# 1dayac/spades_for_blackbird

Hardware: AMD Instinct MI355X
Metric: distinct k-mers/sec (k=21, 150 bp synthetic reads, count only) (higher is better)
Workload: dtype u64

## Files before the change

### spades_for_blackbird_amd/csrc/bbk_internal.h

```cpp
#pragma once

#include <hip/hip_runtime.h>

#include <cstdint>
#include <cstdio>
#include <cstdlib>
#include <map>
#include <memory>
#include <string>
#include <type_traits>
#include <utility>
#include <vector>

#include "../../include/bbk.h"

namespace bbk {

void set_error(const char *fmt, ...);
const char *get_error();

struct Error {
    int code;
};

// ... 97 lines not shown
    int num_cus = 256;
    int num_xcds = 8;
    struct Pending {
        hipEvent_t a, b;
        std::string family;
        double bytes;
    };
    std::vector<Pending> pending;
    std::map<std::string, bbk::FamilyStat> stats;
    void resolve_pending();
    void add_stat(const char *name, double value) {
        if (!profiling) return;
        bbk::FamilyStat &f = stats[name];
        f.launches += 1;
        f.bytes += value;
    }
    void *pinned[2] = {nullptr, nullptr};
    size_t pinned_bytes = 0;
    void *plan_pinned = nullptr;
    size_t plan_pinned_bytes = 0;
    size_t mem_free = 0;
    uint64_t mem_free_mapped_now = ~0ull, mem_free_mapped_total = ~0ull;
    double superk_dup = 0;
};

namespace bbk {

struct KernelTimer {
    bbk_ctx *ctx;
    hipEvent_t a = nullptr, b = nullptr;
    std::string family;
    double bytes;
    KernelTimer(bbk_ctx *c, const char *fam, double algorithmic_bytes = 0) : ctx(c), family(fam), bytes(algorithmic_bytes) {
        if (ctx->profiling) {
            BBK_HIP(hipEventCreate(&a));
            BBK_HIP(hipEventCreate(&b));
            BBK_HIP(hipEventRecord(a, ctx->stream));
        }
    }
    ~KernelTimer() {
        if (a) {
            (void)hipEventRecord(b, ctx->stream);
            ctx->pending.push_back({a, b, family, bytes});
        }
    }
};
// ... 11 lines not shown
                  Args... args) {
    if (lds)
        BBK_HIP(hipFuncSetAttribute(reinterpret_cast<const void *>(fn), hipFuncAttributeMaxDynamicSharedMemorySize,
                                    (int)lds));
    KernelTimer t(ctx, name, bytes);
    hipLaunchKernelGGL(fn, dim3(grid), dim3(threads), lds, ctx->stream, args...);
    check_launch(name);
}

template <class F>
void dispatch_w(unsigned W, F &&f) {
    switch (W) {
        case 1: f(std::integral_constant<int, 1>{}); break;
        case 2: f(std::integral_constant<int, 2>{}); break;
        case 3: f(std::integral_constant<int, 3>{}); break;
        case 4: f(std::integral_constant<int, 4>{}); break;
        default: BBK_REQUIRE(false, BBK_ERR_ARG, "unsupported key width %u", W);
    }
}

inline void stream_wait(bbk_ctx *ctx) {
    ctx->add_stat("stat_host_waits", 1);
    BBK_HIP(hipStreamSynchronize(ctx->stream));
}

inline void d2h_sync(bbk_ctx *ctx, void *dst, const void *src, size_t bytes) {
    BBK_HIP(hipMemcpyAsync(dst, src, bytes, hipMemcpyDeviceToHost, ctx->stream));
    BBK_HIP(hipStreamSynchronize(ctx->stream));
}

inline uint64_t env_u64(const char *v, uint64_t unset) { return v ? strtoull(v, nullptr, 10) : unset; }

inline unsigned words_of(unsigned k) { return (k + 31) >> 5; }

#define BBK_GID() ((((uint64_t)blockIdx.y * gridDim.x) + blockIdx.x) * blockDim.x + threadIdx.x)
inline dim3 grid_blocks(uint64_t blocks) {
    constexpr uint64_t kMaxX = 1ull << 21;
    if (blocks <= kMaxX) return dim3((unsigned)(blocks ? blocks : 1));
    return dim3((unsigned)kMaxX, (unsigned)((blocks + kMaxX - 1) / kMaxX));
}

template <class K, class... Args>
void launch_items(bbk_ctx *ctx, const char *name, K fn, uint64_t n_threads, Args... args) {
    hipLaunchKernelGGL(fn, grid_blocks((n_threads + 255) / 256), dim3(256), 0, ctx->stream, args...);
    check_launch(name);
}
// ... 36 lines not shown
    const uint64_t *d_words = nullptr;
    const uint64_t *d_woff = nullptr;
    const uint32_t *d_len = nullptr;
    bbk::DevBuf own_words, own_woff, own_len;
};

struct bbk_kmerset {
    unsigned k = 0, W = 0;
    unsigned flags = 0;
    uint64_t n = 0;
    uint64_t instances = 0;
    bbk::DevBuf keys;
    bbk::DevBuf counts;
    bool has_counts = false;
    bool sorted = true;
    bool ref_order = false;
};

namespace bbk {

uint64_t exclusive_scan_u64(bbk_ctx *ctx, const uint64_t *in, uint64_t *out, uint64_t n);
void exclusive_scan2_u64(bbk_ctx *ctx, const uint64_t *in0, uint64_t *out0, const uint64_t *in1, uint64_t *out1,
                         uint64_t n, uint64_t totals[2]);
enum { SCAN_U64 = 0, SCAN_U32_FLAGGED = 1, SCAN_SLOT_FILL = 2, SCAN_READ_UNITS = 3 };
struct ScanSrc {
    const void *p;
    uint32_t kind, stride, cap;
    const uint64_t *woff = nullptr;
    uint32_t *unordered = nullptr;
};
void exclusive_scan_enqueue(bbk_ctx *ctx, int narr, const ScanSrc *src, uint64_t *const *out, uint64_t n,
                            uint64_t *d_total, bool tail, std::vector<DevBuf> &keep);

struct ReadPlan {
    DevBuf coff;
    uint64_t kmers = 0, units = 0;
    void run(bbk_ctx *ctx, const bbk_reads *rd, unsigned k, unsigned C, uint32_t *d_unordered);
};

struct PassDesc {
    int kind;
    int word;
    int shift;
    int bits;
    unsigned nb;
};

std::vector<PassDesc> key_passes(unsigned k);

void sort_records(bbk_ctx *ctx, int W, void *keys, void *keys_tmp, uint32_t *vals, uint32_t *vals_tmp, uint64_t n,
                  const std::vector<PassDesc> &passes);
void partition_records(bbk_ctx *ctx, int W, const void *src, void *dst, const uint32_t *vsrc, uint32_t *vdst, uint64_t n,
                       const PassDesc &pd, uint64_t *h_digit_totals = nullptr);
// ... 37 lines not shown
```

### spades_for_blackbird_amd/csrc/block_scan.h

```cpp
#pragma once

#include <hip/hip_runtime.h>

#include <cstdint>

namespace bbk {

constexpr int kThreads = 256;
constexpr int kWaves = kThreads / 64;

__device__ inline uint32_t wave_incl_scan(uint32_t v) {
    const int lane = threadIdx.x & 63;
#pragma unroll
    for (int d = 1; d < 64; d <<= 1) {
        uint32_t t = __shfl_up(v, d, 64);
        if (lane >= d) v += t;
    }
    return v;
}

__device__ inline uint32_t block_excl_scan(uint32_t v, uint32_t *smem_waves , uint32_t *total) {
    const int lane = threadIdx.x & 63, wave = threadIdx.x >> 6;
    uint32_t incl = wave_incl_scan(v);
    if (lane == 63) smem_waves[wave] = incl;
    __syncthreads();
    uint32_t base = 0, tot = 0;
#pragma unroll
    for (int w = 0; w < kWaves; ++w) {
        uint32_t s = smem_waves[w];
        if (w < wave) base += s;
        tot += s;
    }
    __syncthreads();
    *total = tot;
    return base + incl - v;
}

}
```

### spades_for_blackbird_amd/csrc/context.hip

```cpp
#include <hip/hip_runtime.h>

#include <fcntl.h>
#include <unistd.h>

#include <algorithm>
#include <cstdarg>
#include <cstring>

#include "bbk_internal.h"

namespace bbk {

static thread_local char g_err[1024] = "";
void set_error(const char *fmt, ...) {
    va_list ap;
    va_start(ap, fmt);
    vsnprintf(g_err, sizeof(g_err), fmt, ap);
    va_end(ap);
}
const char *get_error() { return g_err; }

hipError_t copy_async(void *dst, const void *src, size_t bytes, hipMemcpyKind kind, hipStream_t stream) {
    if (bytes == 0) return hipSuccess;
    return hipMemcpyAsync(dst, src, bytes, kind, stream);
// ... 150 lines not shown
                (void)hipMemsetAsync(d_mask, 0, 4, c->stream);
                hipLaunchKernelGGL(k_xcd_probe, dim3(4096), dim3(64), 0, c->stream, d_mask);
                if (hipMemcpyAsync(&h_mask, d_mask, 4, hipMemcpyDeviceToHost, c->stream) == hipSuccess &&
                    hipStreamSynchronize(c->stream) == hipSuccess && h_mask)
                    c->num_xcds = __builtin_popcount(h_mask);
                (void)hipFree(d_mask);
            }
            (void)hipGetLastError();
        }
        *out = c;
    });
}

int bbk_ctx_destroy(bbk_ctx *ctx) {
    if (!ctx) return BBK_OK;
    (void)hipSetDevice(ctx->device);
    ctx->resolve_pending();
    if (ctx->stream) (void)hipStreamSynchronize(ctx->stream);
    bbk::pool_trim(ctx->device);
    if (getenv("BBK_VERBOSE")) bbk::pool_report();
    if (ctx->pinned[0]) (void)hipHostFree(ctx->pinned[0]);
    if (ctx->pinned[1]) (void)hipHostFree(ctx->pinned[1]);
    if (ctx->plan_pinned) (void)hipHostFree(ctx->plan_pinned);
    if (ctx->own_stream && ctx->stream) (void)hipStreamDestroy(ctx->stream);
    delete ctx;
    return BBK_OK;
}

int bbk_ctx_set_stream(bbk_ctx *ctx, void *hip_stream) {
    return bbk::guarded([&] {
        BBK_REQUIRE(ctx != nullptr, BBK_ERR_ARG, "bbk_ctx_set_stream: ctx is NULL");
        BBK_HIP(hipSetDevice(ctx->device));
        BBK_HIP(hipStreamSynchronize(ctx->stream));
        if (ctx->own_stream && ctx->stream) BBK_HIP(hipStreamDestroy(ctx->stream));
        ctx->stream = reinterpret_cast<hipStream_t>(hip_stream);
        ctx->own_stream = false;
    });
}

int bbk_ctx_trim(bbk_ctx *ctx) {
    return bbk::guarded([&] {
        BBK_REQUIRE(ctx != nullptr, BBK_ERR_ARG, "bbk_ctx_trim: ctx is NULL");
        BBK_HIP(hipSetDevice(ctx->device));
        BBK_HIP(hipStreamSynchronize(ctx->stream));
        bbk::pool_trim(ctx->device);
    });
// ... 70 lines not shown
```

### spades_for_blackbird_amd/csrc/msd.hip

```cpp
#include <hip/hip_runtime.h>

#include <algorithm>
#include <chrono>
#include <cmath>
#include <cstdio>
#include <cstdlib>
#include <cstring>
#include <optional>
#include <type_traits>
#include <utility>
#include <vector>

#include "bbk_internal.h"
#include "kmer_ops.h"
#include "msd.h"
#include "msd.h"

#include "msd_part.h"
#include "msd_bucket.h"
#include "msd_narrow_a.h"
#include "msd_stage_b.h"

namespace bbk {

// ... 282 lines not shown
        uint64_t *ctl_total() const { return reinterpret_cast<uint64_t *>(ctl_at(kCtlTotal)); }
        uint64_t h_total() const {
            uint64_t t;
            memcpy(&t, h_ctl + kCtlTotal, 8);
            return t;
        }
        ReadSrc S{}, Sh{};
        TileMap M1{}, M2{};
        PartLevel L1{}, L2{};
        DevBuf spill_k, spill_v;
        DevBuf hist1, cur1, bufA, valA;
        uint32_t n32 = 0;
        std::vector<uint32_t> h1, off1, tstart, snb2, sbin, hsub, fill1;
        std::vector<uint32_t> over_seg;
        uint32_t nbuckets = 0, ntiles2 = 0, nwg2 = 0;
        bool narrow_b = false;
        uint32_t *stage = nullptr;
        DevBuf layout_d;
        uint32_t *seg_tile = nullptr, *seg_off = nullptr, *seg_nb2 = nullptr, *seg_bin = nullptr, *seg_size = nullptr,
                 *xstart_d = nullptr;
        DevBuf desc2, desc2h, hist2, boff, bufB, valB;
        std::vector<uint32_t> xstart;
        DevBuf dcount, slot_off, bseg, bbase, flag_ids;
        DevBuf bperm, pfill;
        DevBuf c64, d64;
        bool d64_scanned = false;
        std::vector<DevBuf> scan_keep;
        BucketArgs A{};
        bool direct = false;
        uint32_t ctr[4] = {0, 0, 0, 0};
        std::vector<uint32_t> flagged, hd, hb;
        std::vector<uint32_t> big;
        uint32_t hbo[2] = {0, 0};
        MsdOutput extra;
        uint64_t novf = 0;

        Pass(MsdRunner &r, const MsdInput &i, MsdOutput &o, const Sel &s, Dst d)
            : R(r), ctx(r.ctx), in(i), out(o), sel(s), dst(d), from_reads(i.rd != nullptr),
              has_val(i.with_mask || i.vals != nullptr), ranged(s.span != 0), has_dst(d.keys != nullptr),
              out_vals(r.op != MSD_OP_NONE), need_vbuf(has_val || out_vals), verbose(r.knobs.verbose) {}

        double rec_bytes(uint64_t n) const { return (double)n * (rec + (has_val ? 4 : 0)); }
        uint32_t *vals_or_null(DevBuf &b) const { return has_val ? b.as<uint32_t>() : nullptr; }

        Outcome run(uint64_t *n_records = nullptr) {
            ctl.alloc(kCtlWords * 4);
            BBK_HIP(hipMemsetAsync(ctl.p, 0, kCtlWords * 4, ctx->stream));
// ... 441 lines not shown
                if constexpr (W == 1)
                    R.template launch_part<false, false, false, true>("k_part_l2", (double)N * (rec + 4), nwg2,
                                                                        bufA.as<Key<W>>(), nullptr, M2, L2, nullptr,
                                                                        hist2.as<uint32_t>(), bufB.as<Key<W>>(), nullptr);
            } else {
                R.template scatter_keys<false>(has_val, "k_part_l2", 2.0 * rec_bytes(N), nwg2, bufA.as<Key<W>>(), valA.as<uint32_t>(), M2,
                               L2, hist2.as<uint32_t>(), bufB.as<Key<W>>(), valB.as<uint32_t>());
            }
        }

        std::optional<Outcome> first_pass() {
            dcount.alloc((size_t)nbuckets * 4 + 16);
            A = BucketArgs{boff.as<uint32_t>(), dcount.as<uint32_t>(), nullptr, (int)R.k,
                           verbose ? ctl_at(kCtlDbg) : nullptr, P.slots ? P.cap2 : 0u, P.slots ? P.stride2 : 0u,
                           hist2.as<uint32_t>(), nullptr, nullptr, nullptr, ~0ull, R.knobs.once.hash_max_probes, nullptr};
            direct = (!P.slots || P.kslots) && R.assume_distinct && (R.dmode == MSD_KEYS || R.dmode == MSD_REF) &&
                     !R.knobs.no_direct;
            if (P.kslots) {
                c64.alloc(((size_t)nbuckets + 1) * 8);
                uint64_t *const so = c64.as<uint64_t>();
                slot_off.alloc(((size_t)nbuckets + 1) * 4 + 16);
                if (P.late_tag) {
                    bbase.alloc(((size_t)nbuckets + 1) * 8);
                    bperm.alloc(((size_t)nbuckets + 1) * 4);
                    pfill.alloc(((size_t)nbuckets + 1) * 4);
                    R.launch_plan(k_bucket_base_lt, "k_bucket_base_lt", nbuckets, (const uint32_t *)seg_nb2,
                                  (const uint32_t *)seg_bin, P.nb1, nbuckets, 2 * (int)R.expand_k - 10, (int)R.expand_k,
                                  bbase.as<uint64_t>(), bperm.as<uint32_t>());
                    R.launch_plan(k_lt_fill_perm, "k_lt_fill_perm", nbuckets, hist2.as<uint32_t>(), bperm.as<uint32_t>(),
                                  nbuckets, P.stride2, P.cap2, pfill.as<uint32_t>());
                    const ScanSrc src{pfill.p, SCAN_U32_FLAGGED, 0u, 0u};
                    exclusive_scan_enqueue(ctx, 1, &src, &so, nbuckets, ctl_total(), false, scan_keep);
                    R.launch_plan(k_lt_unperm, "k_lt_unperm", nbuckets, c64.as<uint64_t>(), bperm.as<uint32_t>(), nbuckets,
                                  slot_off.as<uint32_t>());
                } else {
                    const ScanSrc src{hist2.p, SCAN_SLOT_FILL, P.stride2, P.cap2};
                    exclusive_scan_enqueue(ctx, 1, &src, &so, nbuckets, ctl_total(), false, scan_keep);
                    R.launch_plan(k_scan_to_u32, "k_scan_to_u32", (uint64_t)nbuckets + 1, c64.as<uint64_t>(),
                                  (uint64_t)nbuckets, 0ull, (const uint64_t *)ctl_total(), slot_off.as<uint32_t>());
                }
                A.out_off = slot_off.as<uint32_t>();
            }
            if (direct) {
                if (!has_dst) {
                    out.keys.alloc(N * rec + 16);
                    if (out_vals) out.vals.alloc(N * 4 + 16);
                }
                A.sorted_keys = has_dst ? dst.keys : out.keys.p;
                A.sorted_vals = has_dst ? dst.vals : out.vals.as<uint32_t>();
                A.dup_flag = ctl_at(kCtlDup);
                A.strip_mask = R.strip_mask;
            }
            launch_buckets();
            flag_ids.alloc((size_t)kFlagCap * 4);
            if (P.hslots && !direct) {
                d64.alloc(((size_t)nbuckets + 1) * 8);
                const ScanSrc src{dcount.p, SCAN_U32_FLAGGED, 0u, 0u};
                uint64_t *const so = d64.as<uint64_t>();
                exclusive_scan_enqueue(ctx, 1, &src, &so, nbuckets, ctl_total(), false, scan_keep);
                d64_scanned = true;
            }
            fetch_flags();
            if (P.kslots && h_total() != N) {
                if (verbose) fprintf(stderr, "[bbk] msd key slots: %llu of %llu records placed, exact mode\n",
                                     (unsigned long long)h_total(), (unsigned long long)N);
                out.keys.release();
                out.vals.release();
                return give_up_key_slots();
            }
            if (!direct) return std::nullopt;
            if (ctr[2] == 0 && ctr[3] == 0 && (!P.kslots || ctr[0] == 0)) {
                out.n = N;
                out.nbuckets = 0;
                out.overflow_buckets = 0;
                if (P.kslots && verbose)
                    fprintf(stderr, "[bbk] msd key slots N=%llu buckets=%u: ordered without histograms\n",
                            (unsigned long long)N, nbuckets);
                return Outcome::Done;
            }
            if (P.kslots) {
// ... 31 lines not shown
            } else if (narrow_b) {
                if constexpr (W == 1) {
                    BBK_REQUIRE(direct, BBK_ERR_INTERNAL, "4-byte stage-B records need the direct output");
                    if (!P.late_tag) bbase.alloc(((size_t)nbuckets + 1) * 8);
                    if (nbuckets) {
                        if (!P.late_tag)
                            R.launch_plan(k_bucket_base, "k_bucket_base", nbuckets, (const uint32_t *)seg_nb2,
                                          (const uint32_t *)seg_bin, P.nb1, nbuckets, P.b1, R.w0bits(), bbase.as<uint64_t>());
                        constexpr int NT = BktCfg<1>::NT, IT = BktCfg<1>::ITEMS;
                        const bool wide = A.slot_cap != 0 && A.slot_stride % 4 == 0;
                        R.launch(wide ? k_bucket_dist_nb<NT, IT, true> : k_bucket_dist_nb<NT, IT, false>, "k_bucket_dist",
                                 (double)N * (4 + rec), nbuckets, NT, bucket_dist_nb_smem<NT, IT>(), bufB.as<uint32_t>(),
                                 bbase.as<uint64_t>(), A);
                    }
                }
            } else {
                R.template bucket_dispatch<false>(nbuckets, bufB.as<Key<W>>(), valB.as<uint32_t>(), A, rec_bytes(N));
            }
        }

        void fetch_flags() {
            uint32_t *d_flag_n = P.slots ? ctl_at(kCtlSpill) + 2 : ctl_at(kCtlFlagN);
            if (!P.slots) BBK_HIP(hipMemsetAsync(d_flag_n, 0, 16, ctx->stream));
            R.launch_plan(k_flagged, "k_flagged", nbuckets, dcount.as<uint32_t>(), nbuckets, flag_ids.as<uint32_t>(), kFlagCap,
                          d_flag_n);
            BBK_HIP(hipMemcpyAsync(h_ctl, ctl.p, kCtlWords * 4, hipMemcpyDeviceToHost, ctx->stream));
            stream_wait(ctx);
            if (P.slots) memcpy(ctr, h_ctl + kCtlSpill, 12);
            else ctr[2] = h_ctl[kCtlFlagN];
            if (direct) ctr[3] = h_ctl[kCtlDup];
        }

        std::optional<Outcome> overflow() {
            const uint32_t n_flag = ctr[2];
            if (n_flag > kFlagCap) {
                if (verbose) fprintf(stderr, "[bbk] msd: %u buckets overflow\n", n_flag);
                return P.slots ? Outcome::SlotsGaveUp : Outcome::Declined;
            }
            flagged.resize(n_flag);
            if (n_flag) {
                BBK_HIP(hipMemcpyAsync(flagged.data(), flag_ids.p, (size_t)n_flag * 4, hipMemcpyDeviceToHost, ctx->stream));
                stream_wait(ctx);
                std::sort(flagged.begin(), flagged.end());
            }
            const bool exact_check = !P.slots && (n_flag || verbose);
            if (exact_check) {
                hd.resize(nbuckets);
                hb.resize((size_t)nbuckets + 1);
// ... 675 lines not shown
```

### spades_for_blackbird_amd/csrc/msd_part.h

```cpp
#pragma once

namespace bbk {

#ifndef BBK_KEYS_TILE
#define BBK_KEYS_TILE 8192
#endif
#ifndef BBK_KEYS_THREADS
#define BBK_KEYS_THREADS 512
#endif
template <int W>
struct PartCfg {
    static constexpr int TILE = (W == 1) ? BBK_KEYS_TILE : (W == 2 ? 4096 : 2048);
    static constexpr int THREADS = BBK_KEYS_THREADS;
    static constexpr int ITEMS = TILE / THREADS;
};
constexpr int kRdThreads = 1024;
constexpr int kRdHistThreads = 512;
constexpr int kRdSlots = 1024;
constexpr int kRdWords = 2048;
template <int W>
struct RdCfg {
    static constexpr int CH = (W == 1) ? 8 : (W == 2 ? 4 : 2);
    static constexpr int TILE = kRdThreads * CH;
};
// ... 154 lines not shown
        const uint64_t rem = M.n - T.begin;
        T.count = rem < (uint64_t)tile_size ? (uint32_t)rem : tile_size;
        T.nb = L.nb1;
        T.gbin0 = 0;
    }
    return T;
}

#ifdef BBK_PHASE_PROF
__device__ unsigned long long g_phase[6][8];
#define BBK_PH(kind, ph, t_prev)                                                   \
    do {                                                                           \
        if (threadIdx.x == 0) {                                                    \
            const unsigned long long t_now = clock64();                            \
            atomicAdd(&g_phase[kind][ph], t_now - t_prev);                         \
            t_prev = t_now;                                                        \
        }                                                                          \
    } while (0)
#else
#define BBK_PH(kind, ph, t_prev) \
    do {                         \
    } while (0)
#endif

__device__ __forceinline__ uint32_t wave_scan_incl(uint32_t v) {
    v += (uint32_t)__builtin_amdgcn_update_dpp(0, (int)v, 0x111, 0xf, 0xf, false);
    v += (uint32_t)__builtin_amdgcn_update_dpp(0, (int)v, 0x112, 0xf, 0xf, false);
    v += (uint32_t)__builtin_amdgcn_update_dpp(0, (int)v, 0x114, 0xf, 0xf, false);
    v += (uint32_t)__builtin_amdgcn_update_dpp(0, (int)v, 0x118, 0xf, 0xf, false);
    v += (uint32_t)__builtin_amdgcn_update_dpp(0, (int)v, 0x142, 0xa, 0xf, false);
    v += (uint32_t)__builtin_amdgcn_update_dpp(0, (int)v, 0x143, 0xc, 0xf, false);
    return v;
}

template <int NW>
__device__ __forceinline__ void wave_totals(const uint32_t *tmp, int lane, int wave, uint32_t &before, uint32_t &total) {
    static_assert(NW <= 16, "one DPP row");
    const uint32_t v = lane < NW ? tmp[lane] : 0u;
    uint32_t inc = v;
    if (NW > 1) inc += (uint32_t)__builtin_amdgcn_update_dpp(0, (int)inc, 0x111, 0xf, 0xf, false);
    if (NW > 2) inc += (uint32_t)__builtin_amdgcn_update_dpp(0, (int)inc, 0x112, 0xf, 0xf, false);
    if (NW > 4) inc += (uint32_t)__builtin_amdgcn_update_dpp(0, (int)inc, 0x114, 0xf, 0xf, false);
    if (NW > 8) inc += (uint32_t)__builtin_amdgcn_update_dpp(0, (int)inc, 0x118, 0xf, 0xf, false);
    total = (uint32_t)__builtin_amdgcn_readlane((int)inc, NW - 1);
    before = (uint32_t)__builtin_amdgcn_readlane((int)(inc - v), __builtin_amdgcn_readfirstlane(wave));
}

template <int W, int ITEMS, int THREADS, int MAXB, bool HAS_VAL, bool NOUT = false>
__device__ __forceinline__ void part_tail(const Key<W> (&keys)[ITEMS], const uint32_t (&vals)[ITEMS],
                                          const uint32_t (&binrank)[ITEMS], uint32_t *lhist, uint32_t *lstart,
                                          uint32_t *goff, uint32_t *scan_tmp, Key<W> *stage, uint32_t *vstage,
                                          uint32_t nb, uint64_t gbin0, const PartLevel &L,
                                          uint32_t *__restrict__ cursor, Key<W> *__restrict__ out,
                                          uint32_t *__restrict__ vout, int prof_kind = 0,
                                          unsigned long long t_prev = 0) {
    const int tid = threadIdx.x;
// ... 503 lines not shown
```

### spades_for_blackbird_amd/csrc/msd_stage_b.h

```cpp
#pragma once

#include "msd_bucket_tail.h"

namespace bbk {

__global__ void k_bucket_base(const uint32_t *__restrict__ seg_nb2, const uint32_t *__restrict__ seg_bin, uint32_t nseg,
                              uint32_t nbuckets, int b1, int w0bits, uint64_t *__restrict__ base) {
    const uint32_t g = blockIdx.x * blockDim.x + threadIdx.x;
    if (g >= nbuckets) return;
    const uint32_t lo = last_le(seg_bin, nseg, g);
    const uint64_t P = 1ull << (32 - b1), nb = seg_nb2[lo], j = g - seg_bin[lo];
    const uint64_t p = lo * P + (j * P + nb - 1) / nb;
    base[g] = w0bits > 32 ? p << (w0bits - 32) : 0ull;
}

template <int NT, int ITEMS, bool WIDE>
__global__ __launch_bounds__(NT) __attribute__((amdgpu_waves_per_eu(8, 8))) void k_bucket_dist_nb(const uint32_t *__restrict__ buf, const uint64_t *__restrict__ base,
                                                       BucketArgs A) {
    constexpr int CAP = NT * ITEMS;
    constexpr int NWAVES = NT / 64;
    constexpr int DB = DistBins<1, 0>::N;
    constexpr int BPT = DB / NT;
    extern __shared__ __attribute__((aligned(16))) unsigned char smem[];
    uint32_t *bins = reinterpret_cast<uint32_t *>(smem);
// ... 527 lines not shown
    }
#pragma unroll
    for (int i = 0; i < ITEMS; ++i) asm volatile("" : "+v"(lo[i]));
#pragma unroll
    for (int i = 0; i < ITEMS; ++i) {
        Key<1> x;
        x.w[0] = segbits | lo[i];
        const uint32_t tag = (uint32_t)__umul64hi(xxh3_64<1>(x), 16ull);
        const uint32_t b = tag * nsub + __umulhi(lo[i] << (32 - lobits), nsub);
        const bool valid = (uint32_t)i * NT + tid < count;
        if (valid) atomicAdd(&S.lhist[b], 1u);
        const uint32_t b16 = valid ? b : 0xFFFFu;
        if (i & 1) bins[i >> 1] |= b16 << 16;
        else bins[i >> 1] = b16;
    }
    __syncthreads();
    const uint64_t slot_end = (uint64_t)(gbin0 + tid) * L.slot_stride + L.slot_cap;
    mark_tail<NT * ITEMS, ITEMS, false>(
        S, lo, tid, nb, &cursor[gbin0 + tid], slot_end, (uint32_t)segbits, L, out, nullptr,
        [&](int i) { return lt_bin<ITEMS>(bins, i); }, [](int) { return 0u; },
        [&](uint32_t, uint32_t rec) { return lt_tagged(sgm, rec, lobits, k); }, []() {});
}

__global__ void k_bucket_base_lt(const uint32_t *__restrict__ seg_nb2, const uint32_t *__restrict__ seg_bin, uint32_t nseg,
                                 uint32_t nbuckets, int lobits, int k, uint64_t *__restrict__ base,
                                 uint32_t *__restrict__ perm) {
    const uint32_t g = blockIdx.x * blockDim.x + threadIdx.x;
    if (g >= nbuckets) return;
    const uint32_t lo = last_le(seg_bin, nseg, g);
    const uint32_t nsub = seg_nb2[lo] >> 4, r = g - seg_bin[lo], tag = r / nsub, j = r - tag * nsub;
    const uint64_t q = (((uint64_t)j << lobits) + nsub - 1u) / nsub;
    base[g] = ((uint64_t)tag << (2 * k)) | ((uint64_t)lo << lobits) | q;
    perm[g] = tag * (nbuckets >> 4) + (seg_bin[lo] >> 4) + j;
}

__global__ void k_lt_fill_perm(const uint32_t *__restrict__ cursor, const uint32_t *__restrict__ perm, uint32_t n,
                               uint32_t stride, uint32_t cap, uint32_t *__restrict__ fill) {
    const uint32_t g = blockIdx.x * blockDim.x + threadIdx.x;
    if (g >= n) return;
    const uint32_t c = cursor[g] - g * stride;
    fill[perm[g]] = c < cap ? c : cap;
}

__global__ void k_lt_unperm(const uint64_t *__restrict__ scanned, const uint32_t *__restrict__ perm, uint32_t n,
                            uint32_t *__restrict__ out_off) {
    const uint32_t g = blockIdx.x * blockDim.x + threadIdx.x;
    if (g < n) out_off[g] = (uint32_t)scanned[perm[g]];
}

__global__ void k_view_recanon_lt(const uint32_t *__restrict__ in, const uint32_t *__restrict__ seg_off,
                                  const uint32_t *__restrict__ seg_size, int sub_shift, int k, uint64_t *__restrict__ out,
                                  uint64_t cap, uint32_t *__restrict__ count) {
    const uint32_t o = seg_off[blockIdx.x], n = seg_size[blockIdx.x];
    const uint64_t segbits = (uint64_t)(blockIdx.x >> sub_shift) << (2 * k - 10);
    const int lane = threadIdx.x & 63;
    for (uint32_t i0 = 0; i0 < n; i0 += blockDim.x) {
        const uint32_t i = i0 + threadIdx.x;
        Key<1> x;
        x.w[0] = 0;
        bool keep = false;
        if (i < n) {
            x.w[0] = segbits | in[o + i];
            keep = !kmer_less_nucl<1>(kmer_rc<1>(x, k), x);
        }
        const uint64_t bal = __ballot(keep);
        uint32_t base = 0;
        if (lane == 0 && bal) base = atomicAdd(count, (uint32_t)__popcll(bal));
        base = __shfl(base, 0);
        const uint64_t at = (uint64_t)base + __popcll(bal & ((1ull << lane) - 1ull));
        if (keep && at < cap) out[at] = x.w[0];
    }
// ... 20 lines not shown
```

### spades_for_blackbird_amd/csrc/scan.hip

```cpp
#include <hip/hip_runtime.h>

#include <vector>

#include "bbk_internal.h"
#include "block_scan.h"

namespace bbk {

constexpr int kScanItems = 16;
constexpr int kScanTile = kThreads * kScanItems;

struct ScanArrs {
    ScanSrc src[2];
    uint64_t *out[2];
    uint64_t *bsum[2];
    uint64_t *total[2];
    uint64_t *tail[2];
};

__device__ inline uint64_t scan_load(const ScanSrc &s, uint64_t i) {
    if (s.kind == SCAN_U64) return reinterpret_cast<const uint64_t *>(s.p)[i];
    const uint32_t v = reinterpret_cast<const uint32_t *>(s.p)[i];
    if (s.kind == SCAN_U32_FLAGGED) return v == 0xFFFFFFFFu ? 0ull : (uint64_t)v;
    if (s.kind == SCAN_READ_UNITS) {
        const uint32_t c = v >= s.stride ? v - s.stride + 1u : 0u;
        if (c == 0u) return 0ull;
        const uint32_t q = (s.cap & (s.cap - 1u)) ? (c - 1u) / s.cap : (c - 1u) >> (__ffs(s.cap) - 1);
        return (uint64_t)q + 1ull;
    }
    const uint32_t c = v - (uint32_t)i * s.stride;
    return c < s.cap ? c : s.cap;
// ... 80 lines not shown
template <int NA>
static void scan_level(bbk_ctx *ctx, ScanArrs A, uint64_t n, std::vector<DevBuf> &keep) {
    const uint64_t nb = (n + kScanTile - 1) / kScanTile;
    if (nb <= 1) {
        hipLaunchKernelGGL((k_scan_apply<NA, true>), dim3(1), dim3(kThreads), 0, ctx->stream, A, n);
        check_launch("k_scan_apply");
        return;
    }
    BBK_REQUIRE(nb < (1ull << 31), BBK_ERR_ARG, "scan of %llu items", (unsigned long long)n);
    keep.emplace_back((size_t)NA * (nb + 1) * sizeof(uint64_t));
    uint64_t *bs = keep.back().as<uint64_t>();
    ScanArrs B = A;
    for (int a = 0; a < NA; ++a) {
        A.bsum[a] = bs + (size_t)a * (nb + 1);
        B.src[a] = ScanSrc{A.bsum[a], SCAN_U64, 0u, 0u};
        B.out[a] = A.bsum[a];
    }
    hipLaunchKernelGGL((k_scan_reduce<NA>), dim3((unsigned)nb), dim3(kThreads), 0, ctx->stream, A, n);
    check_launch("k_scan_reduce");
    scan_level<NA>(ctx, B, nb, keep);
    hipLaunchKernelGGL((k_scan_apply<NA, false>), dim3((unsigned)nb), dim3(kThreads), 0, ctx->stream, A, n);
    check_launch("k_scan_apply");
}

void exclusive_scan_enqueue(bbk_ctx *ctx, int narr, const ScanSrc *src, uint64_t *const *out, uint64_t n,
                            uint64_t *d_total, bool tail, std::vector<DevBuf> &keep) {
    BBK_REQUIRE(narr == 1 || narr == 2, BBK_ERR_INTERNAL, "scan of %d arrays", narr);
    ScanArrs A{};
    for (int a = 0; a < narr; ++a) {
        A.src[a] = src[a];
        A.out[a] = out[a];
        A.total[a] = d_total + a;
        A.tail[a] = (tail && out[a]) ? out[a] + n : nullptr;
    }
    if (narr == 1) scan_level<1>(ctx, A, n, keep);
    else scan_level<2>(ctx, A, n, keep);
}

uint64_t exclusive_scan_u64(bbk_ctx *ctx, const uint64_t *in, uint64_t *out, uint64_t n) {
    if (n == 0) return 0;
    std::vector<DevBuf> keep;
    keep.reserve(4);
    DevBuf dt(16);
    const ScanSrc src{in, SCAN_U64, 0u, 0u};
    exclusive_scan_enqueue(ctx, 1, &src, &out, n, dt.as<uint64_t>(), false, keep);
    uint64_t total = 0;
// ... 51 lines not shown
```

Before: 33.57 billion.

## Replace multi-launch scan with single-pass decoupled look-back scan and fold scatter/flag steps

Scans of up to 2^24 items now run as one kernel launch that uses a decoupled look-back chain, with ticket-based tile ordering and epoch tags, in place of the reduce, recursive scan and apply launches. The late-tag slot scan now gathers through an inverse permutation and scatters its results directly, which removes the separate unpermute kernel. The flagged-bucket list is emitted during the scan, so the extra k_flagged pass is skipped. This cuts kernel launches and memory passes, at the cost of spin-waiting between tiles, a persistent chain buffer, and a host-mapped give-up flag checked on every stream wait.

Result: no change. 33.78 billion, median of 6 (+0.6%).

```diff
diff --git a/spades_for_blackbird_amd/csrc/bbk_internal.h b/spades_for_blackbird_amd/csrc/bbk_internal.h
--- a/spades_for_blackbird_amd/csrc/bbk_internal.h
+++ b/spades_for_blackbird_amd/csrc/bbk_internal.h
@@ -143,6 +143,10 @@
     size_t mem_free = 0;
     uint64_t mem_free_mapped_now = ~0ull, mem_free_mapped_total = ~0ull;
     double superk_dup = 0;
+    void *scan_chain = nullptr;
+    uint32_t scan_epoch = 0, scan_tickets = 0;
+    volatile uint32_t *scan_gave_up = nullptr;
+    void *scan_gave_up_dev = nullptr;
 };
 
 namespace bbk {
@@ -200,6 +204,10 @@
 inline void stream_wait(bbk_ctx *ctx) {
     ctx->add_stat("stat_host_waits", 1);
     BBK_HIP(hipStreamSynchronize(ctx->stream));
+    if (ctx->scan_gave_up && *ctx->scan_gave_up) {
+        *ctx->scan_gave_up = 0;
+        BBK_REQUIRE(false, BBK_ERR_INTERNAL, "scan: a tile stopped waiting for the tiles before it");
+    }
 }
 
 inline void d2h_sync(bbk_ctx *ctx, void *dst, const void *src, size_t bytes) {
@@ -282,13 +290,21 @@
 uint64_t exclusive_scan_u64(bbk_ctx *ctx, const uint64_t *in, uint64_t *out, uint64_t n);
 void exclusive_scan2_u64(bbk_ctx *ctx, const uint64_t *in0, uint64_t *out0, const uint64_t *in1, uint64_t *out1,
                          uint64_t n, uint64_t totals[2]);
-enum { SCAN_U64 = 0, SCAN_U32_FLAGGED = 1, SCAN_SLOT_FILL = 2, SCAN_READ_UNITS = 3 };
+enum { SCAN_U64 = 0, SCAN_U32_FLAGGED = 1, SCAN_SLOT_FILL = 2, SCAN_READ_UNITS = 3, SCAN_SLOT_FILL_AT = 4 };
 struct ScanSrc {
     const void *p;
     uint32_t kind, stride, cap;
     const uint64_t *woff = nullptr;
     uint32_t *unordered = nullptr;
-};
+    uint32_t *flag_ids = nullptr, *flag_n = nullptr;
+    uint32_t flag_cap = 0;
+    const uint32_t *at = nullptr;
+    uint32_t *out32 = nullptr;
+};
+constexpr uint64_t kScanOneMax = 1ull << 24;
+#if defined(BBK_AB_SCAN_OLD) && !defined(BBK_AB_NO_SCAN_FOLD)
+#define BBK_AB_NO_SCAN_FOLD
+#endif
 void exclusive_scan_enqueue(bbk_ctx *ctx, int narr, const ScanSrc *src, uint64_t *const *out, uint64_t n,
                             uint64_t *d_total, bool tail, std::vector<DevBuf> &keep);
 
diff --git a/spades_for_blackbird_amd/csrc/block_scan.h b/spades_for_blackbird_amd/csrc/block_scan.h
--- a/spades_for_blackbird_amd/csrc/block_scan.h
+++ b/spades_for_blackbird_amd/csrc/block_scan.h
@@ -19,6 +19,16 @@
     return v;
 }
 
+__device__ __forceinline__ uint32_t wave_scan_incl(uint32_t v) {
+    v += (uint32_t)__builtin_amdgcn_update_dpp(0, (int)v, 0x111, 0xf, 0xf, false);
+    v += (uint32_t)__builtin_amdgcn_update_dpp(0, (int)v, 0x112, 0xf, 0xf, false);
+    v += (uint32_t)__builtin_amdgcn_update_dpp(0, (int)v, 0x114, 0xf, 0xf, false);
+    v += (uint32_t)__builtin_amdgcn_update_dpp(0, (int)v, 0x118, 0xf, 0xf, false);
+    v += (uint32_t)__builtin_amdgcn_update_dpp(0, (int)v, 0x142, 0xa, 0xf, false);
+    v += (uint32_t)__builtin_amdgcn_update_dpp(0, (int)v, 0x143, 0xc, 0xf, false);
+    return v;
+}
+
 __device__ inline uint32_t block_excl_scan(uint32_t v, uint32_t *smem_waves , uint32_t *total) {
     const int lane = threadIdx.x & 63, wave = threadIdx.x >> 6;
     uint32_t incl = wave_incl_scan(v);
diff --git a/spades_for_blackbird_amd/csrc/context.hip b/spades_for_blackbird_amd/csrc/context.hip
--- a/spades_for_blackbird_amd/csrc/context.hip
+++ b/spades_for_blackbird_amd/csrc/context.hip
@@ -196,6 +196,8 @@
     if (ctx->pinned[0]) (void)hipHostFree(ctx->pinned[0]);
     if (ctx->pinned[1]) (void)hipHostFree(ctx->pinned[1]);
     if (ctx->plan_pinned) (void)hipHostFree(ctx->plan_pinned);
+    if (ctx->scan_chain) (void)hipFree(ctx->scan_chain);
+    if (ctx->scan_gave_up) (void)hipHostFree((void *)ctx->scan_gave_up);
     if (ctx->own_stream && ctx->stream) (void)hipStreamDestroy(ctx->stream);
     delete ctx;
     return BBK_OK;
diff --git a/spades_for_blackbird_amd/csrc/msd.hip b/spades_for_blackbird_amd/csrc/msd.hip
--- a/spades_for_blackbird_amd/csrc/msd.hip
+++ b/spades_for_blackbird_amd/csrc/msd.hip
@@ -328,7 +328,12 @@
         DevBuf desc2, desc2h, hist2, boff, bufB, valB;
         std::vector<uint32_t> xstart;
         DevBuf dcount, slot_off, bseg, bbase, flag_ids;
+#ifdef BBK_AB_NO_SCAN_FOLD
         DevBuf bperm, pfill;
+#else
+        DevBuf binv;
+        bool flags_listed = false;
+#endif
         DevBuf c64, d64;
         bool d64_scanned = false;
         std::vector<DevBuf> scan_keep;
@@ -816,6 +821,17 @@
                 slot_off.alloc(((size_t)nbuckets + 1) * 4 + 16);
                 if (P.late_tag) {
                     bbase.alloc(((size_t)nbuckets + 1) * 8);
+#ifndef BBK_AB_NO_SCAN_FOLD
+                    binv.alloc(((size_t)nbuckets + 1) * 4);
+                    R.launch_plan(k_bucket_base_lt, "k_bucket_base_lt", nbuckets, (const uint32_t *)seg_nb2,
+                                  (const uint32_t *)seg_bin, P.nb1, nbuckets, 2 * (int)R.expand_k - 10, (int)R.expand_k,
+                                  bbase.as<uint64_t>(), binv.as<uint32_t>());
+                    ScanSrc src{hist2.p, SCAN_SLOT_FILL_AT, P.stride2, P.cap2};
+                    src.at = binv.as<uint32_t>();
+                    src.out32 = slot_off.as<uint32_t>();
+                    uint64_t *const none = nullptr;
+                    exclusive_scan_enqueue(ctx, 1, &src, &none, nbuckets, ctl_total(), false, scan_keep);
+#else
                     bperm.alloc(((size_t)nbuckets + 1) * 4);
                     pfill.alloc(((size_t)nbuckets + 1) * 4);
                     R.launch_plan(k_bucket_base_lt, "k_bucket_base_lt", nbuckets, (const uint32_t *)seg_nb2,
@@ -827,6 +843,7 @@
                     exclusive_scan_enqueue(ctx, 1, &src, &so, nbuckets, ctl_total(), false, scan_keep);
                     R.launch_plan(k_lt_unperm, "k_lt_unperm", nbuckets, c64.as<uint64_t>(), bperm.as<uint32_t>(), nbuckets,
                                   slot_off.as<uint32_t>());
+#endif
                 } else {
                     const ScanSrc src{hist2.p, SCAN_SLOT_FILL, P.stride2, P.cap2};
                     exclusive_scan_enqueue(ctx, 1, &src, &so, nbuckets, ctl_total(), false, scan_keep);
@@ -849,7 +866,13 @@
             flag_ids.alloc((size_t)kFlagCap * 4);
             if (P.hslots && !direct) {
                 d64.alloc(((size_t)nbuckets + 1) * 8);
-                const ScanSrc src{dcount.p, SCAN_U32_FLAGGED, 0u, 0u};
+                ScanSrc src{dcount.p, SCAN_U32_FLAGGED, 0u, 0u};
+#ifndef BBK_AB_NO_SCAN_FOLD
+                src.flag_ids = flag_ids.as<uint32_t>();
+                src.flag_n = ctl_at(kCtlSpill) + 2;
+                src.flag_cap = kFlagCap;
+                flags_listed = true;
+#endif
                 uint64_t *const so = d64.as<uint64_t>();
                 exclusive_scan_enqueue(ctx, 1, &src, &so, nbuckets, ctl_total(), false, scan_keep);
                 d64_scanned = true;
@@ -927,8 +950,15 @@
         void fetch_flags() {
             uint32_t *d_flag_n = P.slots ? ctl_at(kCtlSpill) + 2 : ctl_at(kCtlFlagN);
             if (!P.slots) BBK_HIP(hipMemsetAsync(d_flag_n, 0, 16, ctx->stream));
-            R.launch_plan(k_flagged, "k_flagged", nbuckets, dcount.as<uint32_t>(), nbuckets, flag_ids.as<uint32_t>(), kFlagCap,
-                          d_flag_n);
+#ifndef BBK_AB_NO_SCAN_FOLD
+            const bool listed = flags_listed;
+            flags_listed = false;
+#else
+            const bool listed = false;
+#endif
+            if (!listed)
+                R.launch_plan(k_flagged, "k_flagged", nbuckets, dcount.as<uint32_t>(), nbuckets, flag_ids.as<uint32_t>(),
+                              kFlagCap, d_flag_n);
             BBK_HIP(hipMemcpyAsync(h_ctl, ctl.p, kCtlWords * 4, hipMemcpyDeviceToHost, ctx->stream));
             stream_wait(ctx);
             if (P.slots) memcpy(ctr, h_ctl + kCtlSpill, 12);
diff --git a/spades_for_blackbird_amd/csrc/msd_part.h b/spades_for_blackbird_amd/csrc/msd_part.h
--- a/spades_for_blackbird_amd/csrc/msd_part.h
+++ b/spades_for_blackbird_amd/csrc/msd_part.h
@@ -1,4 +1,6 @@
 #pragma once
+
+#include "block_scan.h"
 
 namespace bbk {
 
@@ -200,16 +202,6 @@
     do {                         \
     } while (0)
 #endif
-
-__device__ __forceinline__ uint32_t wave_scan_incl(uint32_t v) {
-    v += (uint32_t)__builtin_amdgcn_update_dpp(0, (int)v, 0x111, 0xf, 0xf, false);
-    v += (uint32_t)__builtin_amdgcn_update_dpp(0, (int)v, 0x112, 0xf, 0xf, false);
-    v += (uint32_t)__builtin_amdgcn_update_dpp(0, (int)v, 0x114, 0xf, 0xf, false);
-    v += (uint32_t)__builtin_amdgcn_update_dpp(0, (int)v, 0x118, 0xf, 0xf, false);
-    v += (uint32_t)__builtin_amdgcn_update_dpp(0, (int)v, 0x142, 0xa, 0xf, false);
-    v += (uint32_t)__builtin_amdgcn_update_dpp(0, (int)v, 0x143, 0xc, 0xf, false);
-    return v;
-}
 
 template <int NW>
 __device__ __forceinline__ void wave_totals(const uint32_t *tmp, int lane, int wave, uint32_t &before, uint32_t &total) {
diff --git a/spades_for_blackbird_amd/csrc/msd_stage_b.h b/spades_for_blackbird_amd/csrc/msd_stage_b.h
--- a/spades_for_blackbird_amd/csrc/msd_stage_b.h
+++ b/spades_for_blackbird_amd/csrc/msd_stage_b.h
@@ -573,6 +573,7 @@
         [&](uint32_t, uint32_t rec) { return lt_tagged(sgm, rec, lobits, k); }, []() {});
 }
 
+#ifdef BBK_AB_NO_SCAN_FOLD
 __global__ void k_bucket_base_lt(const uint32_t *__restrict__ seg_nb2, const uint32_t *__restrict__ seg_bin, uint32_t nseg,
                                  uint32_t nbuckets, int lobits, int k, uint64_t *__restrict__ base,
                                  uint32_t *__restrict__ perm) {
@@ -598,6 +599,23 @@
     const uint32_t g = blockIdx.x * blockDim.x + threadIdx.x;
     if (g < n) out_off[g] = (uint32_t)scanned[perm[g]];
 }
+#else
+__global__ void k_bucket_base_lt(const uint32_t *__restrict__ seg_nb2, const uint32_t *__restrict__ seg_bin, uint32_t nseg,
+                                 uint32_t nbuckets, int lobits, int k, uint64_t *__restrict__ base,
+                                 uint32_t *__restrict__ inv) {
+    const uint32_t g = blockIdx.x * blockDim.x + threadIdx.x;
+    if (g >= nbuckets) return;
+    {
+        const uint32_t lo = last_le(seg_bin, nseg, g);
+        const uint32_t nsub = seg_nb2[lo] >> 4, r = g - seg_bin[lo], tag = r / nsub, j = r - tag * nsub;
+        const uint64_t q = (((uint64_t)j << lobits) + nsub - 1u) / nsub;
+        base[g] = ((uint64_t)tag << (2 * k)) | ((uint64_t)lo << lobits) | q;
+    }
+    const uint32_t per = nbuckets >> 4, tag = g / per, place = g - tag * per;
+    const uint32_t s = last_le(seg_bin, nseg, place << 4);
+    inv[g] = seg_bin[s] + tag * (seg_nb2[s] >> 4) + (place - (seg_bin[s] >> 4));
+}
+#endif
 
 __global__ void k_view_recanon_lt(const uint32_t *__restrict__ in, const uint32_t *__restrict__ seg_off,
                                   const uint32_t *__restrict__ seg_size, int sub_shift, int k, uint64_t *__restrict__ out,
diff --git a/spades_for_blackbird_amd/csrc/scan.hip b/spades_for_blackbird_amd/csrc/scan.hip
--- a/spades_for_blackbird_amd/csrc/scan.hip
+++ b/spades_for_blackbird_amd/csrc/scan.hip
@@ -7,6 +7,7 @@
 
 namespace bbk {
 
+#ifdef BBK_AB_SCAN_OLD
 constexpr int kScanItems = 16;
 constexpr int kScanTile = kThreads * kScanItems;
 
@@ -133,6 +134,469 @@
     hipLaunchKernelGGL((k_scan_apply<NA, false>), dim3((unsigned)nb), dim3(kThreads), 0, ctx->stream, A, n);
     check_launch("k_scan_apply");
 }
+
+#else
+constexpr int kScanItems = 16;
+constexpr int kScanTile = kThreads * kScanItems;
+constexpr int kScanWaveItems = 64 * kScanItems;
+static_assert(kScanOneMax % kScanTile == 0, "whole tiles");
+constexpr uint32_t kScanOneTiles = (uint32_t)(kScanOneMax / kScanTile);
+
+struct ScanArrs {
+    ScanSrc src[2];
+    uint64_t *out[2];
+    uint64_t *bsum[2];
+    uint64_t *total[2];
+    uint64_t *tail[2];
+};
+
+typedef __attribute__((address_space(1))) unsigned long long gu64;
+typedef __attribute__((address_space(1))) unsigned int gu32;
+
+struct ScanChain {
+    uint32_t ticket;
+    uint32_t pad[3];
+    unsigned long long gran[(size_t)kScanOneTiles * 2 * 2 * 2];
+};
+constexpr uint32_t kScanSpinMax = 1u << 20;
+
+__device__ __forceinline__ void chain_put(ScanChain *c, uint32_t tile, int a, int kind, uint32_t tag, uint64_t v) {
+    gu64 *g = (gu64 *)&c->gran[(((size_t)tile * 2 + a) * 2 + kind) * 2];
+    __hip_atomic_store(g, ((unsigned long long)tag << 32) | (uint32_t)v, __ATOMIC_RELAXED, __HIP_MEMORY_SCOPE_AGENT);
+    __hip_atomic_store(g + 1, ((unsigned long long)tag << 32) | (uint32_t)(v >> 32), __ATOMIC_RELAXED,
+                       __HIP_MEMORY_SCOPE_AGENT);
+}
+__device__ __forceinline__ bool chain_get(ScanChain *c, uint32_t tile, int a, int kind, uint32_t tag, uint64_t &v) {
+    gu64 *g = (gu64 *)&c->gran[(((size_t)tile * 2 + a) * 2 + kind) * 2];
+    const unsigned long long lo = __hip_atomic_load(g, __ATOMIC_RELAXED, __HIP_MEMORY_SCOPE_AGENT);
+    const unsigned long long hi = __hip_atomic_load(g + 1, __ATOMIC_RELAXED, __HIP_MEMORY_SCOPE_AGENT);
+    v = (hi << 32) | (uint32_t)lo;
+    return (uint32_t)(lo >> 32) == tag && (uint32_t)(hi >> 32) == tag;
+}
+
+__device__ __forceinline__ uint64_t wave_sum64(uint64_t v) {
+#pragma unroll
+    for (int d = 32; d >= 1; d >>= 1) v += __shfl_xor(v, d, 64);
+    return v;
+}
+__device__ __forceinline__ uint64_t first_lane64(uint64_t v) {
+    return ((uint64_t)(uint32_t)__builtin_amdgcn_readfirstlane((int)(v >> 32)) << 32) |
+           (uint32_t)__builtin_amdgcn_readfirstlane((int)(uint32_t)v);
+}
+
+template <int NA>
+__device__ __forceinline__ void chain_look_back(ScanChain *c, uint32_t tile, uint32_t epoch, int lane,
+                                                const uint64_t (&own)[NA], uint64_t (&excl)[NA], uint32_t *gave_up) {
+    const uint32_t tag_a = (epoch << 2) | 1u, tag_p = (epoch << 2) | 2u;
+    if (lane == 0) {
+#pragma unroll
+        for (int a = 0; a < NA; ++a) chain_put(c, tile, a, 0, tag_a, own[a]);
+    }
+    uint64_t acc[NA];
+#pragma unroll
+    for (int a = 0; a < NA; ++a) acc[a] = 0;
+    int64_t look = (int64_t)tile - 1;
+    for (uint32_t spins = 0;;) {
+        const int64_t t = look - lane;
+        int st = 2;
+        uint64_t va[NA], vp[NA];
+#pragma unroll
+        for (int a = 0; a < NA; ++a) va[a] = vp[a] = 0;
+        if (t >= 0) {
+            bool has_p = true, has_a = true;
+#pragma unroll
+            for (int a = 0; a < NA; ++a) {
+                has_p &= chain_get(c, (uint32_t)t, a, 1, tag_p, vp[a]);
+                has_a &= chain_get(c, (uint32_t)t, a, 0, tag_a, va[a]);
+            }
+            st = has_p ? 2 : has_a ? 1 : 0;
+        }
+        if (__any(st == 0)) {
+            if (++spins > kScanSpinMax) {
+                if (lane == 0) __hip_atomic_store(gave_up, 1u, __ATOMIC_RELAXED, __HIP_MEMORY_SCOPE_SYSTEM);
+                break;
+            }
+            __builtin_amdgcn_s_sleep(2);
+            continue;
+        }
+        const unsigned long long pm = __ballot(st == 2);
+        const int first = pm ? __ffsll(pm) - 1 : 64;
+#pragma unroll
+        for (int a = 0; a < NA; ++a) {
+            const uint64_t v = lane < first ? va[a] : lane == first ? vp[a] : 0ull;
+            acc[a] += wave_sum64(v);
+        }
+        if (pm) break;
+        look -= 64;
+    }
+#pragma unroll
+    for (int a = 0; a < NA; ++a) {
+        excl[a] = acc[a];
+        if (lane == 0) chain_put(c, tile, a, 1, tag_p, acc[a] + own[a]);
+    }
+}
+
+template <typename VT>
+__device__ __forceinline__ void scan_rows_raw(const ScanSrc &s, uint64_t first, int lane, uint32_t cnt,
+                                              VT (&raw)[kScanItems]) {
+    uint32_t idx[kScanItems];
+#pragma unroll
+    for (int r = 0; r < kScanItems; ++r) {
+        const uint32_t o = (uint32_t)r * 64 + lane;
+        idx[r] = o < cnt ? o : cnt - 1u;
+    }
+    if (sizeof(VT) == 8 && s.kind == SCAN_U64) {
+        const uint64_t *p = reinterpret_cast<const uint64_t *>(s.p) + first;
+#pragma unroll
+        for (int r = 0; r < kScanItems; ++r) raw[r] = (VT)p[idx[r]];
+    } else if (s.kind == SCAN_SLOT_FILL_AT) {
+        const uint32_t *at = s.at + first;
+        uint32_t g[kScanItems];
+#pragma unroll
+        for (int r = 0; r < kScanItems; ++r) g[r] = at[idx[r]];
+#pragma unroll
+        for (int r = 0; r < kScanItems; ++r)
+            raw[r] = reinterpret_cast<const uint32_t *>(s.p)[g[r]] - g[r] * s.stride;
+    } else {
+        const uint32_t *p = reinterpret_cast<const uint32_t *>(s.p) + first;
+#pragma unroll
+        for (int r = 0; r < kScanItems; ++r) raw[r] = p[idx[r]];
+    }
+}
+__device__ __forceinline__ uint64_t scan_value(const ScanSrc &s, uint64_t raw, uint64_t i) {
+    if (s.kind == SCAN_U64) return raw;
+    const uint32_t v = (uint32_t)raw;
+    if (s.kind == SCAN_U32_FLAGGED) return v == 0xFFFFFFFFu ? 0ull : (uint64_t)v;
+    if (s.kind == SCAN_READ_UNITS) {
+        const uint32_t c = v >= s.stride ? v - s.stride + 1u : 0u;
+        if (c == 0u) return 0ull;
+        const uint32_t q = (s.cap & (s.cap - 1u)) ? (c - 1u) / s.cap : (c - 1u) >> (__ffs(s.cap) - 1);
+        return (uint64_t)q + 1ull;
+    }
+    const uint32_t c = s.kind == SCAN_SLOT_FILL_AT ? v : v - (uint32_t)i * s.stride;
+    return c < s.cap ? c : s.cap;
+}
+__device__ __forceinline__ bool scan_same_words(const ScanSrc &a, const ScanSrc &b) {
+    return a.p == b.p && a.kind != SCAN_SLOT_FILL_AT && b.kind != SCAN_SLOT_FILL_AT &&
+           (a.kind == SCAN_U64) == (b.kind == SCAN_U64);
+}
+
+struct ScanOrder {
+    uint64_t w[kScanItems], behind;
+};
+__device__ __forceinline__ void order_load(const ScanSrc &s, uint64_t first, int lane, uint32_t cnt, bool more,
+                                           ScanOrder &o) {
+    const uint64_t *w = s.woff + first;
+#pragma unroll
+    for (int r = 0; r < kScanItems; ++r) {
+        const uint32_t i = (uint32_t)r * 64 + lane;
+        o.w[r] = w[i < cnt ? i : cnt - 1u];
+    }
+    o.behind = w[more ? (uint32_t)kScanWaveItems : cnt - 1u];
+}
+template <typename VT>
+__device__ __forceinline__ bool order_bad(const ScanOrder &o, const VT (&len)[kScanItems], int lane, uint32_t cnt,
+                                          bool more) {
+    const uint32_t pairs = more ? cnt : cnt - 1u;
+    bool bad = false;
+#pragma unroll
+    for (int r = 0; r < kScanItems; ++r) {
+        const uint32_t i = (uint32_t)r * 64 + lane;
+        uint64_t next = __shfl_down(o.w[r], 1, 64);
+        const uint64_t row_next = r + 1 < kScanItems ? first_lane64(o.w[r + 1 < kScanItems ? r + 1 : r]) : o.behind;
+        if (lane == 63) next = row_next;
+        bad |= i < pairs && next < o.w[r] + (((uint32_t)len[r] + 31u) >> 5);
+    }
+    return bad;
+}
+
+template <int NA, bool SIDE, typename VT>
+__device__ __forceinline__ void scan_tile_load(const ScanArrs &A, uint64_t first, int lane, uint64_t n,
+                                               VT (&v)[NA][kScanItems], uint64_t (&sum)[NA], uint32_t skip = 0u) {
+    const bool same = NA == 2 && skip == 0u && scan_same_words(A.src[0], A.src[NA - 1]);
+    VT raw[NA][kScanItems];
+    ScanOrder order;
+    int checked = -1;
+    if (SIDE) {
+#pragma unroll
+        for (int a = 0; a < NA; ++a)
+            if (A.src[a].kind == SCAN_READ_UNITS && A.src[a].woff) checked = a;
+    }
+    const uint32_t cnt = first < n ? (uint32_t)(n - first < (uint64_t)kScanWaveItems ? n - first : kScanWaveItems) : 0u;
+    const bool more = first < n && n - first > (uint64_t)kScanWaveItems;
+    if (cnt) {
+#pragma unroll
+        for (int a = 0; a < NA; ++a) {
+            if ((a == 1 && same) || (skip >> a & 1u)) continue;
+            scan_rows_raw<VT>(A.src[a], first, lane, cnt, raw[a]);
+        }
+        if (SIDE && checked >= 0) order_load(A.src[checked], first, lane, cnt, more, order);
+        if (NA == 2 && same) {
+#pragma unroll
+            for (int r = 0; r < kScanItems; ++r) raw[NA - 1][r] = raw[0][r];
+        }
+    } else {
+#pragma unroll
+        for (int a = 0; a < NA; ++a)
+#pragma unroll
+            for (int r = 0; r < kScanItems; ++r) raw[a][r] = 0;
+    }
+#pragma unroll
+    for (int a = 0; a < NA; ++a) {
+        const ScanSrc &s = A.src[a];
+        sum[a] = 0;
+        const bool on = !(skip >> a & 1u);
+#pragma unroll
+        for (int r = 0; r < kScanItems; ++r) {
+            const uint32_t o = (uint32_t)r * 64 + lane;
+            v[a][r] = on && o < cnt ? (VT)scan_value(s, raw[a][r], first + o) : (VT)0;
+            sum[a] += v[a][r];
+        }
+        if (SIDE && cnt) {
+            if (checked == a) {
+                if (order_bad<VT>(order, raw[a], lane, cnt, more)) *s.unordered = 1u;
+            }
+            if (s.kind == SCAN_U32_FLAGGED && s.flag_n) {
+#pragma unroll
+                for (int r = 0; r < kScanItems; ++r) {
+                    const uint32_t o = (uint32_t)r * 64 + lane;
+                    if (o < cnt && (uint32_t)raw[a][r] == 0xFFFFFFFFu) {
+                        const uint32_t at = atomicAdd(s.flag_n, 1u);
+                        if (at < s.flag_cap) s.flag_ids[at] = (uint32_t)(first + o);
+                    }
+                }
+            }
+        }
+    }
+}
+
+template <typename VT>
+__device__ __forceinline__ void scan_wave_store(const ScanSrc &s, uint64_t *out, const VT (&v)[kScanItems],
+                                                uint64_t first, int lane, uint64_t n, uint64_t run, uint64_t wsum) {
+    const bool narrow = first_lane64(wsum) < (1ull << 32);
+    uint64_t ex[kScanItems];
+    if (narrow) {
+        uint32_t r32 = 0;
+#pragma unroll
+        for (int r = 0; r < kScanItems; ++r) {
+            const uint32_t x = (uint32_t)v[r];
+            const uint32_t inc = wave_scan_incl(x);
+            ex[r] = run + (uint64_t)(r32 + (inc - x));
+            r32 += (uint32_t)__builtin_amdgcn_readlane((int)inc, 63);
+        }
+    } else {
+#pragma unroll
+        for (int r = 0; r < kScanItems; ++r) {
+            uint64_t inc = v[r];
+#pragma unroll
+            for (int d = 1; d < 64; d <<= 1) {
+                const uint64_t t = __shfl_up(inc, d, 64);
+                if (lane >= d) inc += t;
+            }
+            ex[r] = run + (inc - v[r]);
+            run += __shfl(inc, 63, 64);
+        }
+    }
+    const uint32_t cnt = first < n ? (uint32_t)(n - first < (uint64_t)kScanWaveItems ? n - first : kScanWaveItems) : 0u;
+    if (s.kind == SCAN_SLOT_FILL_AT) {
+        const uint32_t *at = s.at + first;
+#pragma unroll
+        for (int r = 0; r < kScanItems; ++r) {
+            const uint32_t o = (uint32_t)r * 64 + lane;
+            if (o < cnt) s.out32[at[o]] = (uint32_t)ex[r];
+        }
+    } else {
+        uint64_t *dst = out + first;
+#pragma unroll
+        for (int r = 0; r < kScanItems; ++r) {
+            const uint32_t o = (uint32_t)r * 64 + lane;
+            if (o < cnt) dst[o] = ex[r];
+        }
+    }
+}
+__device__ __forceinline__ bool scan_stores(const ScanArrs &A, int a) {
+    return A.out[a] != nullptr || A.src[a].kind == SCAN_SLOT_FILL_AT;
+}
+
+template <int NA, typename VT>
+__global__ __launch_bounds__(kThreads) void k_scan_reduce(ScanArrs A, uint64_t n) {
+    __shared__ uint64_t sm[NA][kWaves];
+    const int lane = threadIdx.x & 63, wave = threadIdx.x >> 6;
+    const uint64_t first = (uint64_t)blockIdx.x * kScanTile + (uint64_t)wave * kScanWaveItems;
+    VT v[NA][kScanItems];
+    uint64_t sum[NA];
+    scan_tile_load<NA, true, VT>(A, first, lane, n, v, sum);
+#pragma unroll
+    for (int a = 0; a < NA; ++a) {
+        const uint64_t w = wave_sum64(sum[a]);
+        if (lane == 0) sm[a][wave] = w;
+    }
+    __syncthreads();
+    if (threadIdx.x < NA) {
+        uint64_t t = 0;
+        for (int w = 0; w < kWaves; ++w) t += sm[threadIdx.x][w];
+        A.bsum[threadIdx.x][blockIdx.x] = t;
+    }
+}
+
+template <int NA, typename VT>
+__global__ __launch_bounds__(kThreads) void k_scan_apply(ScanArrs A, uint64_t n) {
+    __shared__ uint64_t sm[NA][kWaves];
+    const int lane = threadIdx.x & 63, wave = threadIdx.x >> 6;
+    const uint64_t first = (uint64_t)blockIdx.x * kScanTile + (uint64_t)wave * kScanWaveItems;
+    uint32_t skip = 0;
+#pragma unroll
+    for (int a = 0; a < NA; ++a) skip |= scan_stores(A, a) ? 0u : 1u << a;
+    VT v[NA][kScanItems];
+    uint64_t sum[NA], wsum[NA];
+    scan_tile_load<NA, false, VT>(A, first, lane, n, v, sum, skip);
+#pragma unroll
+    for (int a = 0; a < NA; ++a) {
+        wsum[a] = wave_sum64(sum[a]);
+        if (lane == 0) sm[a][wave] = wsum[a];
+    }
+    __syncthreads();
+#pragma unroll
+    for (int a = 0; a < NA; ++a) {
+        if (!scan_stores(A, a)) continue;
+        uint64_t run = A.bsum[a][blockIdx.x];
+        for (int w = 0; w < wave; ++w) run += sm[a][w];
+        scan_wave_store<VT>(A.src[a], A.out[a], v[a], first, lane, n, run, wsum[a]);
+    }
+}
+
+template <int NA, typename VT, bool T0>
+__global__ __launch_bounds__(kThreads) void k_scan_one(ScanArrs A, uint64_t n, ScanChain *chain, uint32_t ticket0,
+                                                       uint32_t epoch, uint32_t tiles, uint32_t *gave_up) {
+    __shared__ uint64_t sm[NA][kWaves];
+    __shared__ uint64_t s_excl[NA];
+    __shared__ uint32_t s_tile;
+    const int lane = threadIdx.x & 63, wave = threadIdx.x >> 6;
+    if (threadIdx.x == 0)
+        s_tile = __hip_atomic_fetch_add((gu32 *)&chain->ticket, 1u, __ATOMIC_RELAXED, __HIP_MEMORY_SCOPE_AGENT) - ticket0;
+    __syncthreads();
+    const uint32_t tile = s_tile;
+    if (tile >= tiles) return;
+    const uint64_t first = (uint64_t)tile * kScanTile + (uint64_t)wave * kScanWaveItems;
+    VT v[NA][kScanItems];
+    uint64_t sum[NA], wsum[NA];
+    scan_tile_load<NA, true, VT>(A, first, lane, n, v, sum);
+#pragma unroll
+    for (int a = 0; a < NA; ++a) {
+        wsum[a] = wave_sum64(sum[a]);
+        if (lane == 0) sm[a][wave] = wsum[a];
+    }
+    __syncthreads();
+    uint64_t before[NA], own[NA];
+#pragma unroll
+    for (int a = 0; a < NA; ++a) {
+        before[a] = own[a] = 0;
+#pragma unroll
+        for (int w = 0; w < kWaves; ++w) {
+            const uint64_t t = sm[a][w];
+            if (w < wave) before[a] += t;
+            own[a] += t;
+        }
+    }
+    if (wave == 0) {
+        uint64_t excl[NA];
+        if (tile == 0) {
+#pragma unroll
+            for (int a = 0; a < NA; ++a) {
+                excl[a] = 0;
+                if (lane == 0) chain_put(chain, 0u, a, 1, (epoch << 2) | 2u, own[a]);
+            }
+        } else {
+            chain_look_back<NA>(chain, tile, epoch, lane, own, excl, gave_up);
+        }
+        if (lane == 0) {
+#pragma unroll
+            for (int a = 0; a < NA; ++a) {
+                s_excl[a] = excl[a];
+                if (tile == tiles - 1) {
+                    const uint64_t t = excl[a] + own[a];
+                    *A.total[a] = t;
+                    if (A.tail[a]) *A.tail[a] = t;
+                }
+            }
+        }
+    }
+    __syncthreads();
+#pragma unroll
+    for (int a = 0; a < NA; ++a) {
+        if ((T0 && a == 0) || !scan_stores(A, a)) continue;
+        scan_wave_store<VT>(A.src[a], A.out[a], v[a], first, lane, n, s_excl[a] + before[a], wsum[a]);
+    }
+}
+
+static ScanChain *scan_chain(bbk_ctx *ctx) {
+    if (!ctx->scan_chain) {
+        BBK_HIP(hipMalloc(&ctx->scan_chain, sizeof(ScanChain)));
+        BBK_HIP(hipMemsetAsync(ctx->scan_chain, 0, sizeof(ScanChain), ctx->stream));
+        ctx->scan_epoch = 0;
+        ctx->scan_tickets = 0;
+        BBK_HIP(hipHostMalloc((void **)&ctx->scan_gave_up, 64, hipHostMallocMapped));
+        *ctx->scan_gave_up = 0;
+        BBK_HIP(hipHostGetDevicePointer(&ctx->scan_gave_up_dev, (void *)ctx->scan_gave_up, 0));
+    }
+    return (ScanChain *)ctx->scan_chain;
+}
+
+template <int NA>
+static bool scan_words32(const ScanArrs &A) {
+    for (int a = 0; a < NA; ++a)
+        if (A.src[a].kind == SCAN_U64) return false;
+    return true;
+}
+
+template <int NA>
+static void scan_one(bbk_ctx *ctx, const ScanArrs &A, uint64_t n) {
+    const uint32_t tiles = n ? (uint32_t)((n + kScanTile - 1) / kScanTile) : 1u;
+    BBK_REQUIRE(tiles <= kScanOneTiles, BBK_ERR_INTERNAL, "one-launch scan of %llu items", (unsigned long long)n);
+    ScanChain *chain = scan_chain(ctx);
+    if (++ctx->scan_epoch >= (1u << 30)) {
+        BBK_HIP(hipMemsetAsync(chain->gran, 0, sizeof(chain->gran), ctx->stream));
+        ctx->scan_epoch = 1;
+    }
+    const uint32_t ticket0 = ctx->scan_tickets;
+    ctx->scan_tickets += tiles;
+    const bool w32 = scan_words32<NA>(A);
+    const bool t0 = NA == 2 && w32 && !A.out[0] && A.src[0].kind != SCAN_SLOT_FILL_AT;
+    auto kern = t0    ? k_scan_one<NA, uint32_t, NA == 2>
+                : w32 ? k_scan_one<NA, uint32_t, false>
+                      : k_scan_one<NA, uint64_t, false>;
+    hipLaunchKernelGGL(kern, dim3(tiles), dim3(kThreads), 0, ctx->stream, A, n, chain, ticket0, ctx->scan_epoch, tiles,
+                       (uint32_t *)ctx->scan_gave_up_dev);
+    check_launch("k_scan_one");
+}
+
+template <int NA>
+static void scan_level(bbk_ctx *ctx, ScanArrs A, uint64_t n, std::vector<DevBuf> &keep) {
+    if (n <= kScanOneMax) {
+        scan_one<NA>(ctx, A, n);
+        return;
+    }
+    const uint64_t nb = (n + kScanTile - 1) / kScanTile;
+    BBK_REQUIRE(nb < (1ull << 31), BBK_ERR_ARG, "scan of %llu items", (unsigned long long)n);
+    keep.emplace_back((size_t)NA * (nb + 1) * sizeof(uint64_t));
+    uint64_t *bs = keep.back().as<uint64_t>();
+    ScanArrs B = A;
+    for (int a = 0; a < NA; ++a) {
+        A.bsum[a] = bs + (size_t)a * (nb + 1);
+        B.src[a] = ScanSrc{A.bsum[a], SCAN_U64, 0u, 0u};
+        B.out[a] = A.bsum[a];
+    }
+    const bool w32 = scan_words32<NA>(A);
+    auto reduce = w32 ? k_scan_reduce<NA, uint32_t> : k_scan_reduce<NA, uint64_t>;
+    auto apply = w32 ? k_scan_apply<NA, uint32_t> : k_scan_apply<NA, uint64_t>;
+    hipLaunchKernelGGL(reduce, dim3((unsigned)nb), dim3(kThreads), 0, ctx->stream, A, n);
+    check_launch("k_scan_reduce");
+    scan_level<NA>(ctx, B, nb, keep);
+    hipLaunchKernelGGL(apply, dim3((unsigned)nb), dim3(kThreads), 0, ctx->stream, A, n);
+    check_launch("k_scan_apply");
+}
+
+#endif
 
 void exclusive_scan_enqueue(bbk_ctx *ctx, int narr, const ScanSrc *src, uint64_t *const *out, uint64_t n,
                             uint64_t *d_total, bool tail, std::vector<DevBuf> &keep) {
```
